# Ouranosinc/xclim

Measured on AMD Instinct MI355X. Metric: grid-cells x timesteps / s (tx90p = percentile_doy + threshold_count + missing mask), higher is better.
Workload: dtype f32

## Files before the change

xclim_amd/csrc/common.h:

```cpp
#pragma once
#include <hip/hip_runtime.h>
#include <stdint.h>
#include <stdio.h>
#include <string.h>

#include "../../include/xclim_hip.h"

struct xh_ctx {
  int device;
  hipStream_t stream;
  hipEvent_t ev0, ev1;
  hipStream_t stream2;
  hipEvent_t ev_ready[2], ev_done[2];
  hipStream_t copy_in, copy_out;
  hipEvent_t ev_lane;
  void* scratch;
  size_t scratch_bytes;
  char* scratch_host;
  size_t scratch_head;
  void* retired[16];
  char* retired_host[16];
  int nretired;
  void* big;
  size_t big_bytes;
// ... 10 lines not shown
  do {                                                                                      \
    hipError_t _e = (expr);                                                                 \
    if (_e != hipSuccess) {                                                                 \
      xh_set_error("%s failed: %s (%s:%d)", #expr, hipGetErrorString(_e), __FILE__, __LINE__); \
      (void)hipGetLastError();   \
      return XH_ERR_HIP;                                                                    \
    }                                                                                       \
  } while (0)

#define XH_REQUIRE(cond, code, ...) \
  do {                              \
    if (!(cond)) {                  \
      xh_set_error(__VA_ARGS__);    \
      return (code);                \
    }                               \
  } while (0)

#define XH_LAUNCH_CHECK()                                                                      \
  do {                                                                                         \
    hipError_t _e = hipGetLastError();                                                         \
    if (_e != hipSuccess) {                                                                    \
      xh_set_error("kernel launch failed: %s (%s:%d)", hipGetErrorString(_e), __FILE__, __LINE__); \
      return XH_ERR_HIP;                                                                       \
    }                                                                                          \
  } while (0)

int xh_nanmax_fix(xh_ctx* ctx, const float* x, int64_t T, int64_t C, int64_t st, int64_t sc, int nq, float* out);
int xh_correction_fix(xh_ctx* ctx, const float* ref, const float* hist, int64_t T, int64_t C, int64_t st, int64_t sc, int nq, int kind,
                      float* af, float* hist_q);
int xh_scratch_upload(xh_ctx* ctx, size_t* cursor, const void* host, size_t bytes, void** dptr);
int xh_big_scratch(xh_ctx* ctx, size_t bytes, void** dptr);
int xh_const_rows(xh_ctx* ctx, int64_t elems, const float** nan_row, const float** ninf_row, const float** pinf_row);
int xh_launch_tcount_doy(xh_ctx* ctx, const float* x, int64_t T, int64_t C, int64_t st, int op, const double* table,
                         int64_t tstride, const int32_t* tidx, const int64_t* d_seg, const int64_t* h_seg, int P, int ndoy,
                         int32_t* count_out, int32_t* valid_out);
int xh_qdm_columns(xh_ctx* ctx, const float* xcols, int64_t T, int64_t ncols, int64_t col_stride, const float* af, int64_t af_qs,
                   const double* d_q, int nq, int kind, int interp, int extrap, float* out, int64_t out_cs);
int xh_qdm_sorted_ws(int64_t T, int64_t ncols, size_t* bytes);
int xh_qdm_sorted(xh_ctx* ctx, const float* xcols, int64_t T, int64_t ncols, int64_t col_stride, const float* af, int64_t af_qs,
                  const double* d_q, int nq, int kind, int interp, int extrap, float* out, int64_t out_cs, void* ws);
int xh_qdm_regsort(xh_ctx* ctx, const float* sim, int64_t T, int64_t C, int64_t st, const float* af, int64_t af_qs,
                   const double* d_q, int nq, int kind, int extrap, float* scen, int64_t ost);
int xh_cut_classify(xh_ctx* ctx, const float* sim, int64_t T, int64_t C, int64_t st, const float* gcut, const float* gfac, int ntest,
                    int kind, float* scen, int64_t ost);
int xh_qdm_hist(xh_ctx* ctx, const float* sim, int64_t T, int64_t C, int64_t st, const float* af, int64_t af_qs, const double* d_q,
                int nq, int kind, int extrap, float* scen, int64_t ost);
int xh_tcount_plan(int64_t T, int64_t C, int64_t st, int op, int P, int ndoy, int64_t longest, size_t* lds, int* narrow);
int64_t xh_tcount_meta_slots(int64_t T);
int64_t xh_tcount_slot_of_row(int64_t t);
int xh_tcount_run(xh_ctx* ctx, const float* x, int64_t T, int64_t C, int64_t st, int op, const double* table, int64_t tstride,
                  const uint32_t* meta, int P, int ndoy, int narrow, size_t lds, int32_t* count_out, int32_t* valid_out);
int xh_select_columns(xh_ctx* ctx, const float* xcols, int64_t T, int64_t ncols, int64_t col_stride, const double* d_q,
                      int nq, float* out, int64_t out_cstride, int64_t out_qstride);
int xh_select_columns_lean(xh_ctx* ctx, const float* xcols, int64_t T, int64_t ncols, int64_t col_stride,
                           const double* d_q, int nq, float* out, int64_t out_cstride, int64_t out_qstride);
int xh_select_columns_radix(xh_ctx* ctx, const float* xcols, int64_t T, int64_t ncols, int64_t col_stride, const double* d_q,
                            int nq, float* out, int64_t out_cstride, int64_t out_qstride);
int xh_select_regsort(xh_ctx* ctx, const float* x, int64_t T, int64_t C, int64_t st, const double* d_q, int nq, float* out,
                      int64_t out_cstride, int64_t out_qstride);
int xh_select_hist(xh_ctx* ctx, const float* x, int64_t T, int64_t C, int64_t st, const double* d_q, int nq, float* out,
                   int64_t out_cstride, int64_t out_qstride);
int xh_select_time_major(xh_ctx* ctx, const float* x, int64_t T, int64_t C, int64_t st, const double* d_q, int nq,
                         float* out, int64_t out_cstride, int64_t out_qstride);

__host__ __device__ static inline int64_t cdiv64(int64_t a, int64_t b) { return (a + b - 1) / b; }

#define XH_BLOCK 256

// ... 212 lines not shown
```

xclim_amd/csrc/quantile.hip:

```cpp
#include <stdlib.h>

#include <type_traits>

#include "pdoy.h"

template <typename Getter>
__device__ __forceinline__ double xh_hf_quantile(int L, int n, double q, double alpha, double beta, Getter get) {
  if (L == 1) return (double)get(0);
  if (n < 2) {
    return n == 1 ? (double)get(0) : xh_nan64();
  }
  double nn = (double)n;
  double vi = nn * q + (alpha + q * (1.0 - alpha - beta)) - 1.0;
  if (vi >= nn - 1.0) return (double)get(n - 1);
  if (vi < 0.0) {
    const float v0 = get(0);
    return (v0 - v0 != 0.0f) ? (double)get(n - 1) : (double)v0;
  }
  double prev = floor(vi);
  int ip = (int)prev;
  double gamma = vi - prev;
  float left = get(ip), right = get(ip + 1);
  float diff = right - left;
  double r = (double)left + (double)diff * gamma;
// ... 67 lines not shown
        return xh_key2f(r);
      };
      for (int j = 0; j < nper; ++j) {
        double r = xh_hf_quantile(N, nvalid[v], qs[j], alpha, beta, get);
        out[((int64_t)j * ndoy + d) * C + c + v] = r;
      }
    }
  }
}

__device__ __forceinline__ void ce(uint32_t& a, uint32_t& b) {
  uint32_t lo = a < b ? a : b, hi = a < b ? b : a;
  a = lo;
  b = hi;
}

template <int W>
__device__ __forceinline__ void sort_small(uint32_t (&k)[W]) {
  if (W == 1) return;
  if (W == 2) { ce(k[0], k[1 % W]); return; }
  if (W == 3) { ce(k[0], k[1 % W]); ce(k[1 % W], k[2 % W]); ce(k[0], k[1 % W]); return; }
  if (W == 5) {
    ce(k[0], k[1 % W]); ce(k[3 % W], k[4 % W]); ce(k[2 % W], k[4 % W]); ce(k[2 % W], k[3 % W]); ce(k[0], k[3 % W]);
    ce(k[0], k[2 % W]); ce(k[1 % W], k[4 % W]); ce(k[1 % W], k[3 % W]); ce(k[1 % W], k[2 % W]);
    return;
  }
#pragma unroll
  for (int r = 0; r < W; ++r) {
#pragma unroll
    for (int i = (r & 1); i + 1 < W; i += 2) ce(k[i], k[i + 1]);
  }
}

template <int W, int VEC, bool COUNT = false>
__global__ void __launch_bounds__(XH_BLOCK)
k_pdoy_slide(const float* __restrict__ x, int64_t T, int64_t C, int64_t st, int64_t t_first, int ndoy, int chunk,
             const QTab* __restrict__ qtab, int nper, double* __restrict__ out, int fast, int op = 0,
             const int32_t* __restrict__ doy_period = nullptr, int32_t* __restrict__ cnt_out = nullptr,
             int32_t* __restrict__ valid_out = nullptr) {
  __shared__ QTab s_tab[8 * (W + 1)];
  for (int i = threadIdx.x; i < nper * (W + 1); i += XH_BLOCK) s_tab[i] = qtab[i];
  __syncthreads();
  constexpr int NP = VEC == 4 ? 2 : 1;
  constexpr int GW = VEC == 4 ? 2 : 1;
  const int lane = threadIdx.x & 63;
  const int64_t wbase = ((int64_t)blockIdx.x * XH_BLOCK + (threadIdx.x & ~63)) * VEC;
  if (wbase >= C) return;
  int64_t cg[NP];
  bool okg[NP];
#pragma unroll
  for (int g = 0; g < NP; ++g) {
    cg[g] = wbase + (VEC == 4 ? 2 * lane + 128 * g : lane);
    okg[g] = cg[g] < C;
  }
  auto cell = [&](int v) -> int64_t { return cg[v / GW] + v % GW; };
  constexpr int half = W / 2;
  int d0 = blockIdx.y * chunk, d1 = d0 + chunk;
  if (d1 > ndoy) d1 = ndoy;
  uint32_t win[VEC][W];
  int n[VEC];
#pragma unroll
  for (int v = 0; v < VEC; ++v) {
    n[v] = 0;
#pragma unroll
    for (int k = 0; k < W; ++k) win[v][k] = 0xFFFFFFFFu;
  }
  auto fetch = [&](int64_t t) -> VecF<VEC> {
    const int64_t tc = t < 0 ? 0 : (t >= T ? T - 1 : t);
    const float* row = x + tc * st;
    VecF<VEC> r;
#pragma unroll
    for (int g = 0; g < NP; ++g) {
      const VecF<GW> h = xh_load<GW>(row + (okg[g] ? cg[g] : C - GW));
#pragma unroll
// ... 499 lines not shown
    hipLaunchKernelGGL((k_pdoy_reg<16, 1>), grid, dim3(XH_BLOCK), 0, ctx->stream, x, T, C, st, d_tbase, nyears, ndoy,
                       window, d_q, nper, alpha, beta, out);
  } else if (N <= 32) {
    dim3 grid((unsigned)cdiv64(C, XH_BLOCK), gy);
    hipLaunchKernelGGL((k_pdoy_reg<32, 1>), grid, dim3(XH_BLOCK), 0, ctx->stream, x, T, C, st, d_tbase, nyears, ndoy,
                       window, d_q, nper, alpha, beta, out);
  } else {
    return launch_pdoy_lds(ctx, x, T, C, st, d_tbase, nyears, ndoy, window, d_q, nper, alpha, beta, out, nullptr, T, nullptr,
                           0);
  }
  XH_LAUNCH_CHECK();
  return XH_OK;
}

static int slide_fast_mode(const QTab* tab, int nper, int W) {
  bool allmax = W > 1, allmin = W > 1;
  for (int j = 0; j < nper; ++j) {
    const QTab& e = tab[j * (W + 1) + W];
    allmax = allmax && e.lo == e.hi && e.lo == W - 1;
    allmin = allmin && e.lo == e.hi && e.lo == 0;
  }
  return allmax ? 1 : (allmin ? 2 : 0);
}

static int pdoy_impl(xh_ctx* ctx, const float* x, int64_t T, int64_t C, int64_t st, const int32_t* tbase, int nyears,
                     int ndoy, int window, const double* qh, int nper, double alpha, double beta, const int32_t* vmap,
                     int64_t Tv, double* out) {
  size_t cur = 0;
  void *d_tb = nullptr, *d_q = nullptr, *d_vmap = nullptr;
  const int N = nyears * window;
  bool contiguous = !vmap && nyears == 1 && nper <= 8 && (window == 3 || window == 5 || window == 7) && tbase[0] >= 0;
  for (int d = 1; contiguous && d < ndoy; ++d) contiguous = tbase[d] == tbase[0] + d;
  if (contiguous) {
    QTab tab[8 * 8];
    build_qtab(window, qh, nper, alpha, beta, tab);
    void* d_tab = nullptr;
    int rc = xh_scratch_upload(ctx, &cur, tab, sizeof(QTab) * (size_t)nper * (window + 1), &d_tab);
    if (rc) return rc;
    int chunk = 32;
    if (const char* e = xh_diag_env("XH_PDOY_SLIDE_CHUNK")) chunk = atoi(e) > 0 ? atoi(e) : chunk;
    const int vec = slide_vec(x, C, st, out);
    dim3 grid((unsigned)cdiv64(cdiv64(C, vec), XH_BLOCK), (unsigned)((ndoy + chunk - 1) / chunk));
#define XH_SLIDE(W, V)                                                                                              \
  hipLaunchKernelGGL((k_pdoy_slide<W, V>), grid, dim3(XH_BLOCK), 0, ctx->stream, x, T, C, st, (int64_t)tbase[0], ndoy, \
                     chunk, (const QTab*)d_tab, nper, out, slide_fast_mode(tab, nper, window))
    if (vec == 4) {
      if (window == 3) XH_SLIDE(3, 4); else if (window == 5) XH_SLIDE(5, 4); else XH_SLIDE(7, 4);
    } else {
      if (window == 3) XH_SLIDE(3, 1); else if (window == 5) XH_SLIDE(5, 1); else XH_SLIDE(7, 1);
    }
#undef XH_SLIDE
    XH_LAUNCH_CHECK();
    return XH_OK;
  }
  int rc = xh_scratch_upload(ctx, &cur, tbase, sizeof(int32_t) * (size_t)nyears * ndoy, &d_tb);
  if (rc) return rc;
  rc = xh_scratch_upload(ctx, &cur, qh, sizeof(double) * nper, &d_q);
  if (rc) return rc;
  if (vmap) {
    rc = xh_scratch_upload(ctx, &cur, vmap, sizeof(int32_t) * (size_t)Tv, &d_vmap);
    if (rc) return rc;
  }
  if (!vmap && N <= 32)
    return launch_pdoy(ctx, x, T, C, st, (const int32_t*)d_tb, nyears, ndoy, window, (const double*)d_q, nper, alpha, beta,
                       out);
  const bool mergeable = N > 32 && nyears <= 64 && (window == 3 || window == 5 || window == 7) && nper <= 16;
  if (!mergeable)
    return launch_pdoy_lds(ctx, x, T, C, st, (const int32_t*)d_tb, nyears, ndoy, window, (const double*)d_q, nper, alpha,
                           beta, out, (const int32_t*)d_vmap, Tv, nullptr, 0);
  uint8_t* regular = (uint8_t*)malloc((size_t)ndoy);
  int32_t* irregular = (int32_t*)malloc(sizeof(int32_t) * (size_t)ndoy);
  QTab* tab = (QTab*)malloc(sizeof(QTab) * (size_t)nper * (N + 1));
  if (!regular || !irregular || !tab) {
    free(regular); free(irregular); free(tab);
    xh_set_error("xh_percentile_doy: out of host memory");
    return XH_ERR_ARG;
  }
  const int nirr = pdoy_regular_flags(tbase, nyears, ndoy, window, T, vmap, Tv, regular, irregular);
// ... 76 lines not shown
                                         hipFuncAttributeMaxDynamicSharedMemorySize, (int)lds));                           \
      hipLaunchKernelGGL((k_pdoy_merge<W, NY, false>), grid, dim3(64), lds, ctx->stream, x, T, C, st, (const int32_t*)d_tb, \
                         nyears, ndoy, chunk, (const QTab*)d_tab, (const int32_t*)d_jrest, nrest, out,                      \
                         (const int32_t*)d_vmap, Tv, (const uint8_t*)d_reg, (const int32_t*)nullptr, 0, KT, KB, abl);       \
    }                                                                                                                      \
    if (nirr) {                                                                                                            \
      if (lds_a > 64 * 1024)                                                                                               \
        XH_CHECK_HIP(hipFuncSetAttribute((const void*)k_pdoy_merge<W, NY, true>,                                           \
                                         hipFuncAttributeMaxDynamicSharedMemorySize, (int)lds_a));                         \
      hipLaunchKernelGGL((k_pdoy_merge<W, NY, true>), grid_irr, dim3(64), lds_a, ctx->stream, x, T, C, st,                  \
                         (const int32_t*)d_tb, nyears, ndoy, chunk, (const QTab*)d_tab, (const int32_t*)d_jall, nper, out,  \
                         (const int32_t*)d_vmap, Tv, (const uint8_t*)d_reg, (const int32_t*)d_irr, nirr, KTa, KBa, abl);    \
    }                                                                                                                      \
  } while (0)
  if (NYP == 32) {
    if (window == 3) XH_MERGE(3, 32); else if (window == 5) XH_MERGE(5, 32); else XH_MERGE(7, 32);
  } else {
    if (window == 3) XH_MERGE(3, 64); else if (window == 5) XH_MERGE(5, 64); else XH_MERGE(7, 64);
  }
#undef XH_MERGE
  XH_LAUNCH_CHECK();
  return XH_OK;
}

static int pdoy_count_impl(xh_ctx* ctx, const float* x, int64_t T, int64_t C, int64_t st, const int32_t* tbase, int ndoy,
                           int window, double per, double alpha, double beta, int op, const int32_t* doy_period, int P,
                           int32_t* count_out, int32_t* valid_out) {
  bool contiguous = (window == 3 || window == 5 || window == 7) && tbase[0] >= 0;
  for (int d = 1; contiguous && d < ndoy; ++d) contiguous = tbase[d] == tbase[0] + d;
  if (!contiguous) return XH_ERR_NOTIMPL;
  for (int d = 0; d < ndoy; ++d)
    XH_REQUIRE(doy_period[d] >= 0 && doy_period[d] < P, XH_ERR_ARG, "xh_percentile_doy_count: doy_period[%d] outside [0, P)", d);
  size_t cur = 0;
  QTab tab[8];
  const double q = per / 100.0;
  build_qtab(window, &q, 1, alpha, beta, tab);
  void *d_tab = nullptr, *d_dp = nullptr;
  int rc = xh_scratch_upload(ctx, &cur, tab, sizeof(QTab) * (size_t)(window + 1), &d_tab);
  if (!rc) rc = xh_scratch_upload(ctx, &cur, doy_period, sizeof(int32_t) * (size_t)ndoy, &d_dp);
  if (rc) return rc;
  XH_CHECK_HIP(hipMemsetAsync(count_out, 0, sizeof(int32_t) * (size_t)P * (size_t)C, ctx->stream));
  if (valid_out) XH_CHECK_HIP(hipMemsetAsync(valid_out, 0, sizeof(int32_t) * (size_t)P * (size_t)C, ctx->stream));
  int chunk = 61;
  if (const char* e = xh_diag_env("XH_PDOY_SLIDE_COUNT_CHUNK")) chunk = atoi(e) > 0 ? atoi(e) : chunk;
  const int vec = slide_vec(x, C, st, nullptr);
  dim3 grid((unsigned)cdiv64(cdiv64(C, vec), XH_BLOCK), (unsigned)((ndoy + chunk - 1) / chunk));
#define XH_SLIDEC(W, V)                                                                                                   \
  hipLaunchKernelGGL((k_pdoy_slide<W, V, true>), grid, dim3(XH_BLOCK), 0, ctx->stream, x, T, C, st, (int64_t)tbase[0], ndoy, \
                     chunk, (const QTab*)d_tab, 1, (double*)nullptr, slide_fast_mode(tab, 1, window), op,          \
                     (const int32_t*)d_dp, count_out, valid_out)
  if (vec == 4) {
    if (window == 3) XH_SLIDEC(3, 4); else if (window == 5) XH_SLIDEC(5, 4); else XH_SLIDEC(7, 4);
  } else {
    if (window == 3) XH_SLIDEC(3, 1); else if (window == 5) XH_SLIDEC(5, 1); else XH_SLIDEC(7, 1);
  }
#undef XH_SLIDEC
  XH_LAUNCH_CHECK();
  return XH_OK;
}

static int pdoy_count_multi(xh_ctx* ctx, const float* x, int64_t T, int64_t C, int64_t st, const int32_t* tbase, int nyears,
                            int ndoy, int window, double per, double alpha, double beta, int op, const int32_t* doy_period,
                            int P, int32_t* count_out, int32_t* valid_out) {
  const int N = nyears * window;
  if (!(N > 32 && nyears <= 64 && (window == 3 || window == 5 || window == 7))) return XH_ERR_NOTIMPL;
  if (op != XH_OP_GT && op != XH_OP_GE && op != XH_OP_LT && op != XH_OP_LE) return XH_ERR_NOTIMPL;
  for (int64_t i = 0; i < (int64_t)nyears * ndoy; ++i) {
    XH_REQUIRE(tbase[i] >= -1 && tbase[i] < T, XH_ERR_ARG, "xh_percentile_doy_count: tbase entry out of range");
    XH_REQUIRE(tbase[i] < 0 ? doy_period[i] < 0 : (doy_period[i] >= 0 && doy_period[i] < P), XH_ERR_ARG,
               "xh_percentile_doy_count: doy_period[%lld] must be in [0, P) for present days and < 0 for absent ones",
               (long long)i);
  }
  uint8_t* regular = (uint8_t*)malloc((size_t)ndoy);
  int32_t* irregular = (int32_t*)malloc(sizeof(int32_t) * (size_t)ndoy);
  QTab* tab = (QTab*)malloc(sizeof(QTab) * (size_t)(N + 1));
  if (!regular || !irregular || !tab) {
    free(regular); free(irregular); free(tab);
    xh_set_error("xh_percentile_doy_count: out of host memory");
    return XH_ERR_ARG;
  }
  const int nirr = pdoy_regular_flags(tbase, nyears, ndoy, window, T, nullptr, T, regular, irregular);
  const double q = per / 100.0;
// ... 188 lines not shown
```

xclim_amd/csrc/reduce.hip:

```cpp
#include "common.h"
#include "window.h"

template <int VEC, int KIND>
__global__ void __launch_bounds__(XH_BLOCK)
k_threshold_count(const float* __restrict__ x, int64_t C, int64_t st, int op, float thr32, double thr64,
                  const void* __restrict__ table, int64_t tstride, const int32_t* __restrict__ tidx,
                  const int64_t* __restrict__ seg_off, int P, int32_t* __restrict__ count_out,
                  int32_t* __restrict__ valid_out, int period_fast) {
  const unsigned tile = period_fast ? blockIdx.y : blockIdx.x;
  const int pstart = period_fast ? blockIdx.x : blockIdx.y, pstep = period_fast ? gridDim.x : gridDim.y;
  int64_t c = ((int64_t)tile * XH_BLOCK + threadIdx.x) * VEC;
  if (c >= C) return;
  for (int p = pstart; p < P; p += pstep) {
    int64_t t0 = seg_off[p], t1 = seg_off[p + 1];
    int cnt[VEC], val[VEC];
#pragma unroll
    for (int i = 0; i < VEC; ++i) cnt[i] = 0, val[i] = 0;
    xh_march_rows<VEC, 8>(x + c, st, t0, t1, [&](int64_t t, const VecF<VEC>& xv) {
      if (KIND == XH_THR_SCALAR_F32) {
#pragma unroll
        for (int i = 0; i < VEC; ++i) cnt[i] += xh_cmp_f32(xv.v[i], op, thr32) ? 1 : 0;
      } else if (KIND == XH_THR_SCALAR_F64) {
#pragma unroll
        for (int i = 0; i < VEC; ++i) cnt[i] += xh_cmp_f64((double)xv.v[i], op, thr64) ? 1 : 0;
// ... 170 lines not shown
        else if (RED == XH_RED_VAR) r = (poisoned || n[i] == 0) ? xh_nan32() : (float)(s2[i] / (double)n[i]);
        else r = (poisoned || n[i] == 0) ? xh_nan32() : (float)sqrt(s2[i] / (double)n[i]);
        if (len == 0 && RED != XH_RED_SUM) r = xh_nan32();
        reinterpret_cast<float*>(out_v)[o + i] = r;
      }
    }
    if (valid_out) {
#pragma unroll
      for (int i = 0; i < VEC; ++i) valid_out[o + i] = n[i];
    }
  }
}

template <int VEC>
static int launch_resample_reduce(xh_ctx* ctx, int reducer, dim3 grid, const float* x, int64_t C, int64_t st, int skipna,
                                  const int64_t* seg, int P, void* out, int32_t* valid_out) {
#define XH_RR(R)                                                                                                   \
  case R:                                                                                                          \
    hipLaunchKernelGGL((k_resample_reduce<VEC, R>), grid, dim3(XH_BLOCK), 0, ctx->stream, x, C, st, skipna, seg, P, out, \
                       valid_out);                                                                                 \
    break;
  switch (reducer) {
    XH_RR(XH_RED_SUM) XH_RR(XH_RED_MEAN) XH_RR(XH_RED_MIN) XH_RR(XH_RED_MAX) XH_RR(XH_RED_STD) XH_RR(XH_RED_VAR)
    XH_RR(XH_RED_COUNT) XH_RR(XH_RED_ARGMIN) XH_RR(XH_RED_ARGMAX)
    default:
      xh_set_error("xh_resample_reduce: reducer %d not recognized", reducer);
      return XH_ERR_OP;
  }
#undef XH_RR
  XH_LAUNCH_CHECK();
  return XH_OK;
}

__global__ void __launch_bounds__(XH_BLOCK)
k_apply_missing_mask(const void* __restrict__ value, int kind, const int32_t* __restrict__ valid,
                     const int32_t* __restrict__ expected, int P, int64_t C, double* __restrict__ out) {
  int64_t i = (int64_t)blockIdx.x * XH_BLOCK + threadIdx.x;
  int64_t n = (int64_t)P * C;
  if (i >= n) return;
  int p = (int)(i / C);
  double v = kind == 0 ? (double)reinterpret_cast<const int32_t*>(value)[i]
             : kind == 1 ? (double)reinterpret_cast<const float*>(value)[i]
                         : reinterpret_cast<const double*>(value)[i];
  out[i] = (valid[i] != expected[p]) ? xh_nan64() : v;
}

template <int RED>
__global__ void __launch_bounds__(XH_BLOCK)
k_rolling_reduce(const float* __restrict__ x, int64_t T, int64_t C, int64_t st, int window, int left, int right,
                 float* __restrict__ out, int64_t out_st) {
  int64_t c = (int64_t)blockIdx.x * XH_BLOCK + threadIdx.x;
  if (c >= C) return;
  int64_t chunk = cdiv64(T, (int64_t)gridDim.y);
  int64_t ta = (int64_t)blockIdx.y * chunk, tb = ta + chunk;
  if (tb > T) tb = T;
  for (int64_t t = ta; t < tb; ++t) {
    int64_t a = t - left, b = t + right;
    float r;
    if (RED == XH_RED_COUNT) {
      int n = 0;
      for (int64_t k = (a < 0 ? 0 : a); k <= b && k < T; ++k) {
        float v = x[k * st + c];
        n += (v == v) ? 1 : 0;
      }
      r = (float)n;
    } else if (a < 0 || b >= T) {
      r = xh_nan32();
    } else {
      double s = 0.0;
      float e = x[a * st + c];
      bool nan = false;
      for (int64_t k = a; k <= b; ++k) {
        float v = x[k * st + c];
        nan |= (v != v);
        if (RED == XH_RED_MIN) e = v < e ? v : e;
        else if (RED == XH_RED_MAX) e = v > e ? v : e;
        else s += (double)v;
      }
      if (RED == XH_RED_SUM) r = (float)s;
      else if (RED == XH_RED_MEAN) r = (float)(s / (double)window);
      else if (RED == XH_RED_MIN || RED == XH_RED_MAX) r = e;
      else {
        double m = s / (double)window, s2 = 0.0;
        for (int64_t k = a; k <= b; ++k) {
          double d = (double)x[k * st + c] - m;
          s2 += d * d;
        }
        r = (RED == XH_RED_VAR) ? (float)(s2 / (double)window) : (float)sqrt(s2 / (double)window);
      }
      if (nan) r = xh_nan32();
    }
    out[t * out_st + c] = r;
  }
}

static int check_tc(const char* fn, xh_ctx* ctx, const void* x, int64_t T, int64_t C, int64_t st, int64_t sc) {
  XH_REQUIRE(ctx && x, XH_ERR_ARG, "%s: NULL argument", fn);
  XH_REQUIRE(T >= 0 && C >= 0, XH_ERR_ARG, "%s: negative shape", fn);
  XH_REQUIRE(sc == 1 && st >= C, XH_ERR_LAYOUT,
             "%s: streaming kernels need a time-major view (sc == 1, st >= C); got st=%lld sc=%lld — transpose first",
             fn, (long long)st, (long long)sc);
  return XH_OK;
}

static int upload_segments(xh_ctx* ctx, size_t* cur, const int64_t* seg_off, int P, int64_t T, const char* fn,
                           const int64_t** d_seg) {
  XH_REQUIRE(seg_off && P >= 1, XH_ERR_ARG, "%s: seg_off NULL or P < 1", fn);
  for (int p = 0; p < P; ++p)
    XH_REQUIRE(seg_off[p] <= seg_off[p + 1] && seg_off[p] >= 0 && seg_off[p + 1] <= T, XH_ERR_ARG,
               "%s: seg_off must be non-decreasing within [0, T]", fn);
  void* d = nullptr;
  int rc = xh_scratch_upload(ctx, cur, seg_off, sizeof(int64_t) * (size_t)(P + 1), &d);
  if (rc) return rc;
  *d_seg = (const int64_t*)d;
  return XH_OK;
}

extern "C" {

static int threshold_count_impl(xh_ctx* ctx, const float* x, int64_t T, int64_t C, int64_t st, int64_t sc, int op, int thr_kind,
                                double thr_scalar, const void* thr_table, int64_t thr_stride, const int32_t* tidx,
                                const int64_t* seg_off, int P, int32_t* count_out, int32_t* valid_out, int ndoy) {
  int rc = check_tc("xh_threshold_count", ctx, x, T, C, st, sc);
  if (rc) return rc;
  XH_REQUIRE(op >= XH_OP_GT && op <= XH_OP_NE, XH_ERR_OP, "Operation `%d` not recognized.", op);
  XH_REQUIRE(count_out, XH_ERR_ARG, "xh_threshold_count: count_out is NULL");
  if (thr_kind >= XH_THR_DOY_F64) {
    XH_REQUIRE(thr_table && thr_stride >= C, XH_ERR_ARG, "xh_threshold_count: threshold table missing or stride < C");
    if (thr_kind == XH_THR_DOY_F64 || thr_kind == XH_THR_DOY_F32)
      XH_REQUIRE(tidx, XH_ERR_ARG, "xh_threshold_count: tidx required for per-doy thresholds");
  }
  size_t cur = 0;
  const int64_t* d_seg = nullptr;
  rc = upload_segments(ctx, &cur, seg_off, P, T, "xh_threshold_count", &d_seg);
  if (rc) return rc;
  if (C == 0) return XH_OK;
  if (thr_kind == XH_THR_DOY_F64 && ndoy > 0 && !xh_diag_env("XH_TCOUNT_LEGACY")) {
    rc = xh_launch_tcount_doy(ctx, x, T, C, st, op, static_cast<const double*>(thr_table), thr_stride, tidx, d_seg, seg_off, P,
                              ndoy, count_out, valid_out);
    if (rc != XH_ERR_NOTIMPL) return rc;
  }
  int vec = xh_pick_vec(x, C, st);
  if (thr_kind >= XH_THR_DOY_F64) {
    size_t esz = (thr_kind == XH_THR_DOY_F64 || thr_kind == XH_THR_FULL_F64) ? 8 : 4;
    if ((reinterpret_cast<uintptr_t>(thr_table) & 15) != 0 || (thr_stride * esz) % 16 != 0) vec = 1;
  }
  unsigned tiles = (unsigned)cdiv64(cdiv64(C, vec), XH_BLOCK);
  const bool doy = thr_kind == XH_THR_DOY_F64 || thr_kind == XH_THR_DOY_F32;
  const int period_fast = (doy && P > 1 && tiles <= 65535u) ? 1 : 0;
  dim3 grid = period_fast ? dim3(period_grid(P), tiles) : dim3(tiles, period_grid(P));
  if (vec == 4)
    return launch_threshold_count<4>(ctx, thr_kind, grid, x, C, st, op, thr_scalar, thr_table, thr_stride, tidx, d_seg, P,
                                     count_out, valid_out, period_fast);
  return launch_threshold_count<1>(ctx, thr_kind, grid, x, C, st, op, thr_scalar, thr_table, thr_stride, tidx, d_seg, P,
                                   count_out, valid_out, period_fast);
}

int xh_threshold_count(xh_ctx* ctx, const float* x, int64_t T, int64_t C, int64_t st, int64_t sc, int op, int thr_kind,
                       double thr_scalar, const void* thr_table, int64_t thr_stride, const int32_t* tidx,
                       const int64_t* seg_off, int P, int32_t* count_out, int32_t* valid_out) {
  return threshold_count_impl(ctx, x, T, C, st, sc, op, thr_kind, thr_scalar, thr_table, thr_stride, tidx, seg_off, P, count_out,
                              valid_out, 0);
}

int xh_threshold_count_doy(xh_ctx* ctx, const float* x, int64_t T, int64_t C, int64_t st, int64_t sc, int op,
                           const double* thr_table, int64_t thr_stride, int ndoy, const int32_t* tidx, const int64_t* seg_off,
                           int P, int32_t* count_out, int32_t* valid_out) {
  XH_REQUIRE(ndoy >= 1, XH_ERR_ARG, "xh_threshold_count_doy: the table needs at least one row (ndoy = %d)", ndoy);
  return threshold_count_impl(ctx, x, T, C, st, sc, op, XH_THR_DOY_F64, 0.0, thr_table, thr_stride, tidx, seg_off, P, count_out,
                              valid_out, ndoy);
}

int xh_domain_count(xh_ctx* ctx, const float* x, int64_t T, int64_t C, int64_t st, int64_t sc, int op1, double thr1,
                    int op2, double thr2, int combine, const int64_t* seg_off, int P, int32_t* count_out,
// ... 19 lines not shown
    hipLaunchKernelGGL((k_domain_count<4, true>), grid, dim3(XH_BLOCK), 0, ctx->stream, x, C, st, s1, c1.thr, s2, c2.thr, combine,
                       d_seg, P, count_out, valid_out);
  } else if (vec == 4)
    hipLaunchKernelGGL((k_domain_count<4>), grid, dim3(XH_BLOCK), 0, ctx->stream, x, C, st, op1, (float)thr1, op2,
                       (float)thr2, combine, d_seg, P, count_out, valid_out);
  else
    hipLaunchKernelGGL((k_domain_count<1>), grid, dim3(XH_BLOCK), 0, ctx->stream, x, C, st, op1, (float)thr1, op2,
                       (float)thr2, combine, d_seg, P, count_out, valid_out);
  XH_LAUNCH_CHECK();
  return XH_OK;
}

int xh_resample_reduce(xh_ctx* ctx, const float* x, int64_t T, int64_t C, int64_t st, int64_t sc, int reducer, int skipna,
                       const int64_t* seg_off, int P, void* out, int32_t* valid_out) {
  int rc = check_tc("xh_resample_reduce", ctx, x, T, C, st, sc);
  if (rc) return rc;
  XH_REQUIRE(out, XH_ERR_ARG, "xh_resample_reduce: out is NULL");
  size_t cur = 0;
  const int64_t* d_seg = nullptr;
  rc = upload_segments(ctx, &cur, seg_off, P, T, "xh_resample_reduce", &d_seg);
  if (rc) return rc;
  if (C == 0) return XH_OK;
  int vec = xh_pick_vec(x, C, st);
  dim3 grid((unsigned)cdiv64(cdiv64(C, vec), XH_BLOCK), period_grid(P));
  if (vec == 4) return launch_resample_reduce<4>(ctx, reducer, grid, x, C, st, skipna, d_seg, P, out, valid_out);
  return launch_resample_reduce<1>(ctx, reducer, grid, x, C, st, skipna, d_seg, P, out, valid_out);
}

int xh_apply_missing_mask(xh_ctx* ctx, const void* value, int value_kind, const int32_t* valid, const int32_t* expected,
                          int P, int64_t C, double* out64) {
  XH_REQUIRE(ctx && value && valid && expected && out64, XH_ERR_ARG, "xh_apply_missing_mask: NULL argument");
  XH_REQUIRE(value_kind >= 0 && value_kind <= 2, XH_ERR_ARG, "xh_apply_missing_mask: value_kind must be 0, 1 or 2");
  XH_REQUIRE(P >= 1 && C >= 0, XH_ERR_ARG, "xh_apply_missing_mask: bad shape");
  size_t cur = 0;
  void* d_exp = nullptr;
  int rc = xh_scratch_upload(ctx, &cur, expected, sizeof(int32_t) * (size_t)P, &d_exp);
  if (rc) return rc;
  int64_t n = (int64_t)P * C;
  if (n == 0) return XH_OK;
  hipLaunchKernelGGL(k_apply_missing_mask, dim3((unsigned)cdiv64(n, XH_BLOCK)), dim3(XH_BLOCK), 0, ctx->stream, value,
                     value_kind, valid, (const int32_t*)d_exp, P, C, out64);
  XH_LAUNCH_CHECK();
  return XH_OK;
}

int xh_rolling_reduce(xh_ctx* ctx, const float* x, int64_t T, int64_t C, int64_t st, int64_t sc, int window, int center,
                      int reducer, float* out, int64_t out_st) {
  int rc = check_tc("xh_rolling_reduce", ctx, x, T, C, st, sc);
  if (rc) return rc;
  XH_REQUIRE(out && out_st >= C, XH_ERR_ARG, "xh_rolling_reduce: out NULL or out_st < C");
  XH_REQUIRE(window >= 1, XH_ERR_ARG, "xh_rolling_reduce: window must be >= 1");
  if (T == 0 || C == 0) return XH_OK;
  int left = center ? window / 2 : window - 1;
  int right = window - 1 - left;
  {
    int rr = xh_launch_rolling_ring(ctx, x, T, C, st, window, left, right, reducer, out, out_st);
    if (rr != XH_ERR_NOTIMPL) return rr;
  }
  unsigned ny = (unsigned)(T < 64 ? T : 64);
  dim3 grid((unsigned)cdiv64(C, XH_BLOCK), ny);
#define XH_RO(R)                                                                                                      \
  case R:                                                                                                             \
    hipLaunchKernelGGL((k_rolling_reduce<R>), grid, dim3(XH_BLOCK), 0, ctx->stream, x, T, C, st, window, left, right, out, \
                       out_st);                                                                                       \
    break;
  switch (reducer) {
    XH_RO(XH_RED_SUM) XH_RO(XH_RED_MEAN) XH_RO(XH_RED_MIN) XH_RO(XH_RED_MAX) XH_RO(XH_RED_STD) XH_RO(XH_RED_VAR)
    XH_RO(XH_RED_COUNT)
    default:
      xh_set_error("xh_rolling_reduce: reducer %d not recognized", reducer);
      return XH_ERR_OP;
  }
#undef XH_RO
  XH_LAUNCH_CHECK();
// ... 5 lines not shown
```

xclim_amd/csrc/tcount.hip:

```cpp
#include "f32thr.h"
#include "rowstream.h"

namespace {

constexpr int TC_CW = 64, TC_RL = 16, TC_U = 16, TC_NT = TC_CW * TC_RL, TC_ROWS = TC_RL * TC_U;

__global__ void k_tc_meta(const int32_t* __restrict__ tidx, const int64_t* __restrict__ seg, int P, int64_t T, int64_t nslots,
                          int ndoy, uint32_t* __restrict__ meta) {
  const int64_t i = (int64_t)blockIdx.x * blockDim.x + threadIdx.x;
  if (i >= nslots) return;
  const int64_t kb = i >> 8;
  const int rl = (int)(i >> 4) & 15, u = (int)i & 15;
  const int64_t t = kb * TC_ROWS + u * TC_RL + rl;
  uint32_t dy = (uint32_t)ndoy, per = (uint32_t)P;
  if (t < T) {
    const int d = tidx[t];
    if (d >= 0 && d < ndoy) dy = (uint32_t)d;
    if (t >= seg[0] && t < seg[P]) {
      int lo = 0, hi = P;
      while (hi - lo > 1) {
        const int mid = (lo + hi) >> 1;
        if (seg[mid] <= t) lo = mid; else hi = mid;
      }
      per = (uint32_t)lo;
// ... 115 lines not shown

int64_t xh_tcount_slot_of_row(int64_t t) {
  const int64_t kb = t / TC_ROWS, r = t % TC_ROWS;
  return (kb * TC_RL + r % TC_RL) * TC_U + r / TC_RL;
}

int xh_tcount_run(xh_ctx* ctx, const float* x, int64_t T, int64_t C, int64_t st, int op, const double* table, int64_t tstride,
                  const uint32_t* meta, int P, int ndoy, int narrow, size_t lds, int32_t* count_out, int32_t* valid_out) {
  const int64_t ntiles = cdiv64(C, TC_CW);
  const unsigned grid = (unsigned)(ntiles < ctx->num_cu ? ntiles : ctx->num_cu);
#define XH_TCD2(OPV, NW)                                                                                                      \
  {                                                                                                                           \
    XH_CHECK_HIP(hipFuncSetAttribute((const void*)k_tc_doy<OPV, NW>, hipFuncAttributeMaxDynamicSharedMemorySize, (int)lds)); \
    hipLaunchKernelGGL((k_tc_doy<OPV, NW>), dim3(grid), dim3(TC_NT), lds, ctx->stream, x, (int)T, C, st, table, tstride, meta,  \
                       ndoy, P, count_out, valid_out);                                                                        \
  }
#define XH_TCD(OPV)                         \
  case OPV:                                 \
    if (narrow) XH_TCD2(OPV, true) else XH_TCD2(OPV, false) \
    break;
  switch (op) {
    XH_TCD(XH_OP_GT)
    XH_TCD(XH_OP_LT)
    XH_TCD(XH_OP_GE)
    XH_TCD(XH_OP_LE)
  }
#undef XH_TCD2
#undef XH_TCD
  XH_LAUNCH_CHECK();
  return XH_OK;
}

int xh_launch_tcount_doy(xh_ctx* ctx, const float* x, int64_t T, int64_t C, int64_t st, int op, const double* table,
                         int64_t tstride, const int32_t* tidx, const int64_t* d_seg, const int64_t* h_seg, int P, int ndoy,
                         int32_t* count_out, int32_t* valid_out) {
  int64_t longest = 0;
  for (int p = 0; p < P; ++p) longest = h_seg[p + 1] - h_seg[p] > longest ? h_seg[p + 1] - h_seg[p] : longest;
  size_t lds = 0;
  int narrow = 0;
  int rc = xh_tcount_plan(T, C, st, op, P, ndoy, longest, &lds, &narrow);
  if (rc) return rc;
  const int64_t nslots = xh_tcount_meta_slots(T);
  void* scratch = nullptr;
  rc = xh_big_scratch(ctx, (size_t)nslots * 4, &scratch);
  if (rc) return rc;
  uint32_t* meta = static_cast<uint32_t*>(scratch);
  hipLaunchKernelGGL(k_tc_meta, dim3((unsigned)cdiv64(nslots, 256)), dim3(256), 0, ctx->stream, tidx, d_seg, P, T, nslots, ndoy, meta);
  return xh_tcount_run(ctx, x, T, C, st, op, table, tstride, meta, P, ndoy, narrow, lds, count_out, valid_out);
}
```

Before: 229.7 billion.

## Pass small tables as kernel arguments and add streaming per-year threshold count kernel

Small quantile tables and the expected-count array for the missing mask are now passed by value as kernel arguments instead of being uploaded to scratch memory. Segment offsets are uploaded only inside the doy tcount path. A new fallback kernel counts threshold exceedances by streaming rows in double-buffered batches with segment bounds held in kernel arguments. The aim is to remove host-to-device uploads and sync overhead on small inputs and to give a faster fallback when the LDS-based doy kernel declines. In exchange, kernel argument size grows and more specialised kernel variants are built.

```diff
diff --git a/xclim_amd/csrc/common.h b/xclim_amd/csrc/common.h
--- a/xclim_amd/csrc/common.h
+++ b/xclim_amd/csrc/common.h
@@ -66,8 +66,8 @@
 int xh_big_scratch(xh_ctx* ctx, size_t bytes, void** dptr);
 int xh_const_rows(xh_ctx* ctx, int64_t elems, const float** nan_row, const float** ninf_row, const float** pinf_row);
 int xh_launch_tcount_doy(xh_ctx* ctx, const float* x, int64_t T, int64_t C, int64_t st, int op, const double* table,
-                         int64_t tstride, const int32_t* tidx, const int64_t* d_seg, const int64_t* h_seg, int P, int ndoy,
-                         int32_t* count_out, int32_t* valid_out);
+                         int64_t tstride, const int32_t* tidx, const int64_t* h_seg, int P, int ndoy, int32_t* count_out,
+                         int32_t* valid_out);
 int xh_qdm_columns(xh_ctx* ctx, const float* xcols, int64_t T, int64_t ncols, int64_t col_stride, const float* af, int64_t af_qs,
                    const double* d_q, int nq, int kind, int interp, int extrap, float* out, int64_t out_cs);
 int xh_qdm_sorted_ws(int64_t T, int64_t ncols, size_t* bytes);
diff --git a/xclim_amd/csrc/quantile.hip b/xclim_amd/csrc/quantile.hip
--- a/xclim_amd/csrc/quantile.hip
+++ b/xclim_amd/csrc/quantile.hip
@@ -123,14 +123,18 @@
   }
 }
 
+struct SlideTab {
+  QTab e[8 * 8];
+};
+
 template <int W, int VEC, bool COUNT = false>
 __global__ void __launch_bounds__(XH_BLOCK)
 k_pdoy_slide(const float* __restrict__ x, int64_t T, int64_t C, int64_t st, int64_t t_first, int ndoy, int chunk,
-             const QTab* __restrict__ qtab, int nper, double* __restrict__ out, int fast, int op = 0,
+             const SlideTab qtab, int nper, double* __restrict__ out, int fast, int op = 0,
              const int32_t* __restrict__ doy_period = nullptr, int32_t* __restrict__ cnt_out = nullptr,
              int32_t* __restrict__ valid_out = nullptr) {
   __shared__ QTab s_tab[8 * (W + 1)];
-  for (int i = threadIdx.x; i < nper * (W + 1); i += XH_BLOCK) s_tab[i] = qtab[i];
+  for (int i = threadIdx.x; i < nper * (W + 1); i += XH_BLOCK) s_tab[i] = qtab.e[i];
   __syncthreads();
   constexpr int NP = VEC == 4 ? 2 : 1;
   constexpr int GW = VEC == 4 ? 2 : 1;
@@ -696,18 +700,17 @@
   bool contiguous = !vmap && nyears == 1 && nper <= 8 && (window == 3 || window == 5 || window == 7) && tbase[0] >= 0;
   for (int d = 1; contiguous && d < ndoy; ++d) contiguous = tbase[d] == tbase[0] + d;
   if (contiguous) {
-    QTab tab[8 * 8];
+    SlideTab st8;
+    memset(&st8, 0, sizeof(st8));
+    QTab* tab = st8.e;
     build_qtab(window, qh, nper, alpha, beta, tab);
-    void* d_tab = nullptr;
-    int rc = xh_scratch_upload(ctx, &cur, tab, sizeof(QTab) * (size_t)nper * (window + 1), &d_tab);
-    if (rc) return rc;
     int chunk = 32;
     if (const char* e = xh_diag_env("XH_PDOY_SLIDE_CHUNK")) chunk = atoi(e) > 0 ? atoi(e) : chunk;
     const int vec = slide_vec(x, C, st, out);
     dim3 grid((unsigned)cdiv64(cdiv64(C, vec), XH_BLOCK), (unsigned)((ndoy + chunk - 1) / chunk));
 #define XH_SLIDE(W, V)                                                                                              \
   hipLaunchKernelGGL((k_pdoy_slide<W, V>), grid, dim3(XH_BLOCK), 0, ctx->stream, x, T, C, st, (int64_t)tbase[0], ndoy, \
-                     chunk, (const QTab*)d_tab, nper, out, slide_fast_mode(tab, nper, window))
+                     chunk, st8, nper, out, slide_fast_mode(tab, nper, window))
     if (vec == 4) {
       if (window == 3) XH_SLIDE(3, 4); else if (window == 5) XH_SLIDE(5, 4); else XH_SLIDE(7, 4);
     } else {
@@ -850,12 +853,13 @@
   for (int d = 0; d < ndoy; ++d)
     XH_REQUIRE(doy_period[d] >= 0 && doy_period[d] < P, XH_ERR_ARG, "xh_percentile_doy_count: doy_period[%d] outside [0, P)", d);
   size_t cur = 0;
-  QTab tab[8];
+  SlideTab st8;
+  memset(&st8, 0, sizeof(st8));
+  QTab* tab = st8.e;
   const double q = per / 100.0;
   build_qtab(window, &q, 1, alpha, beta, tab);
-  void *d_tab = nullptr, *d_dp = nullptr;
-  int rc = xh_scratch_upload(ctx, &cur, tab, sizeof(QTab) * (size_t)(window + 1), &d_tab);
-  if (!rc) rc = xh_scratch_upload(ctx, &cur, doy_period, sizeof(int32_t) * (size_t)ndoy, &d_dp);
+  void* d_dp = nullptr;
+  int rc = xh_scratch_upload(ctx, &cur, doy_period, sizeof(int32_t) * (size_t)ndoy, &d_dp);
   if (rc) return rc;
   XH_CHECK_HIP(hipMemsetAsync(count_out, 0, sizeof(int32_t) * (size_t)P * (size_t)C, ctx->stream));
   if (valid_out) XH_CHECK_HIP(hipMemsetAsync(valid_out, 0, sizeof(int32_t) * (size_t)P * (size_t)C, ctx->stream));
@@ -865,7 +869,7 @@
   dim3 grid((unsigned)cdiv64(cdiv64(C, vec), XH_BLOCK), (unsigned)((ndoy + chunk - 1) / chunk));
 #define XH_SLIDEC(W, V)                                                                                                   \
   hipLaunchKernelGGL((k_pdoy_slide<W, V, true>), grid, dim3(XH_BLOCK), 0, ctx->stream, x, T, C, st, (int64_t)tbase[0], ndoy, \
-                     chunk, (const QTab*)d_tab, 1, (double*)nullptr, slide_fast_mode(tab, 1, window), op,          \
+                     chunk, st8, 1, (double*)nullptr, slide_fast_mode(tab, 1, window), op,          \
                      (const int32_t*)d_dp, count_out, valid_out)
   if (vec == 4) {
     if (window == 3) XH_SLIDEC(3, 4); else if (window == 5) XH_SLIDEC(5, 4); else XH_SLIDEC(7, 4);
diff --git a/xclim_amd/csrc/reduce.hip b/xclim_amd/csrc/reduce.hip
--- a/xclim_amd/csrc/reduce.hip
+++ b/xclim_amd/csrc/reduce.hip
@@ -226,9 +226,14 @@
   return XH_OK;
 }
 
+#define XH_MASK_SMALL 64
+struct XhMaskExp {
+  int32_t v[XH_MASK_SMALL];
+};
 __global__ void __launch_bounds__(XH_BLOCK)
 k_apply_missing_mask(const void* __restrict__ value, int kind, const int32_t* __restrict__ valid,
-                     const int32_t* __restrict__ expected, int P, int64_t C, double* __restrict__ out) {
+                     const int32_t* __restrict__ expected, const XhMaskExp exp_small, int P, int64_t C,
+                     double* __restrict__ out) {
   int64_t i = (int64_t)blockIdx.x * XH_BLOCK + threadIdx.x;
   int64_t n = (int64_t)P * C;
   if (i >= n) return;
@@ -236,7 +241,8 @@
   double v = kind == 0 ? (double)reinterpret_cast<const int32_t*>(value)[i]
              : kind == 1 ? (double)reinterpret_cast<const float*>(value)[i]
                          : reinterpret_cast<const double*>(value)[i];
-  out[i] = (valid[i] != expected[p]) ? xh_nan64() : v;
+  const int32_t e = expected ? expected[p] : exp_small.v[p];
+  out[i] = (valid[i] != e) ? xh_nan64() : v;
 }
 
 template <int RED>
@@ -297,18 +303,28 @@
   return XH_OK;
 }
 
-static int upload_segments(xh_ctx* ctx, size_t* cur, const int64_t* seg_off, int P, int64_t T, const char* fn,
-                           const int64_t** d_seg) {
+static int check_segments(const int64_t* seg_off, int P, int64_t T, const char* fn) {
   XH_REQUIRE(seg_off && P >= 1, XH_ERR_ARG, "%s: seg_off NULL or P < 1", fn);
   for (int p = 0; p < P; ++p)
     XH_REQUIRE(seg_off[p] <= seg_off[p + 1] && seg_off[p] >= 0 && seg_off[p + 1] <= T, XH_ERR_ARG,
                "%s: seg_off must be non-decreasing within [0, T]", fn);
+  return XH_OK;
+}
+
+static int upload_segments(xh_ctx* ctx, size_t* cur, const int64_t* seg_off, int P, int64_t T, const char* fn,
+                           const int64_t** d_seg) {
+  int rc = check_segments(seg_off, P, T, fn);
+  if (rc) return rc;
   void* d = nullptr;
-  int rc = xh_scratch_upload(ctx, cur, seg_off, sizeof(int64_t) * (size_t)(P + 1), &d);
+  rc = xh_scratch_upload(ctx, cur, seg_off, sizeof(int64_t) * (size_t)(P + 1), &d);
   if (rc) return rc;
   *d_seg = (const int64_t*)d;
   return XH_OK;
 }
+
+__attribute__((weak)) int xh_launch_tcount_year(xh_ctx* ctx, const float* x, int64_t T, int64_t C, int64_t st, int op,
+                                                const double* table, int64_t tstride, const int32_t* tidx,
+                                                const int64_t* seg_off, int P, int32_t* count_out, int32_t* valid_out);
 
 extern "C" {
 
@@ -324,16 +340,24 @@
     if (thr_kind == XH_THR_DOY_F64 || thr_kind == XH_THR_DOY_F32)
       XH_REQUIRE(tidx, XH_ERR_ARG, "xh_threshold_count: tidx required for per-doy thresholds");
   }
+  rc = check_segments(seg_off, P, T, "xh_threshold_count");
+  if (rc) return rc;
+  if (C == 0) return XH_OK;
+  const bool legacy = xh_diag_env("XH_TCOUNT_LEGACY") != nullptr;
+  if (thr_kind == XH_THR_DOY_F64 && ndoy > 0 && !legacy) {
+    rc = xh_launch_tcount_doy(ctx, x, T, C, st, op, static_cast<const double*>(thr_table), thr_stride, tidx, seg_off, P, ndoy,
+                              count_out, valid_out);
+    if (rc != XH_ERR_NOTIMPL) return rc;
+  }
+  if (thr_kind == XH_THR_DOY_F64 && !legacy && xh_launch_tcount_year) {
+    rc = xh_launch_tcount_year(ctx, x, T, C, st, op, static_cast<const double*>(thr_table), thr_stride, tidx, seg_off, P,
+                               count_out, valid_out);
+    if (rc != XH_ERR_NOTIMPL) return rc;
+  }
   size_t cur = 0;
   const int64_t* d_seg = nullptr;
   rc = upload_segments(ctx, &cur, seg_off, P, T, "xh_threshold_count", &d_seg);
   if (rc) return rc;
-  if (C == 0) return XH_OK;
-  if (thr_kind == XH_THR_DOY_F64 && ndoy > 0 && !xh_diag_env("XH_TCOUNT_LEGACY")) {
-    rc = xh_launch_tcount_doy(ctx, x, T, C, st, op, static_cast<const double*>(thr_table), thr_stride, tidx, d_seg, seg_off, P,
-                              ndoy, count_out, valid_out);
-    if (rc != XH_ERR_NOTIMPL) return rc;
-  }
   int vec = xh_pick_vec(x, C, st);
   if (thr_kind >= XH_THR_DOY_F64) {
     size_t esz = (thr_kind == XH_THR_DOY_F64 || thr_kind == XH_THR_FULL_F64) ? 8 : 4;
@@ -419,14 +443,20 @@
   XH_REQUIRE(ctx && value && valid && expected && out64, XH_ERR_ARG, "xh_apply_missing_mask: NULL argument");
   XH_REQUIRE(value_kind >= 0 && value_kind <= 2, XH_ERR_ARG, "xh_apply_missing_mask: value_kind must be 0, 1 or 2");
   XH_REQUIRE(P >= 1 && C >= 0, XH_ERR_ARG, "xh_apply_missing_mask: bad shape");
-  size_t cur = 0;
+  XhMaskExp small;
+  memset(&small, 0, sizeof(small));
   void* d_exp = nullptr;
-  int rc = xh_scratch_upload(ctx, &cur, expected, sizeof(int32_t) * (size_t)P, &d_exp);
-  if (rc) return rc;
+  if (P <= XH_MASK_SMALL) {
+    memcpy(small.v, expected, sizeof(int32_t) * (size_t)P);
+  } else {
+    size_t cur = 0;
+    int rc = xh_scratch_upload(ctx, &cur, expected, sizeof(int32_t) * (size_t)P, &d_exp);
+    if (rc) return rc;
+  }
   int64_t n = (int64_t)P * C;
   if (n == 0) return XH_OK;
   hipLaunchKernelGGL(k_apply_missing_mask, dim3((unsigned)cdiv64(n, XH_BLOCK)), dim3(XH_BLOCK), 0, ctx->stream, value,
-                     value_kind, valid, (const int32_t*)d_exp, P, C, out64);
+                     value_kind, valid, (const int32_t*)d_exp, small, P, C, out64);
   XH_LAUNCH_CHECK();
   return XH_OK;
 }
diff --git a/xclim_amd/csrc/tcount.hip b/xclim_amd/csrc/tcount.hip
--- a/xclim_amd/csrc/tcount.hip
+++ b/xclim_amd/csrc/tcount.hip
@@ -171,19 +171,23 @@
 }
 
 int xh_launch_tcount_doy(xh_ctx* ctx, const float* x, int64_t T, int64_t C, int64_t st, int op, const double* table,
-                         int64_t tstride, const int32_t* tidx, const int64_t* d_seg, const int64_t* h_seg, int P, int ndoy,
-                         int32_t* count_out, int32_t* valid_out) {
+                         int64_t tstride, const int32_t* tidx, const int64_t* h_seg, int P, int ndoy, int32_t* count_out,
+                         int32_t* valid_out) {
   int64_t longest = 0;
   for (int p = 0; p < P; ++p) longest = h_seg[p + 1] - h_seg[p] > longest ? h_seg[p + 1] - h_seg[p] : longest;
   size_t lds = 0;
   int narrow = 0;
   int rc = xh_tcount_plan(T, C, st, op, P, ndoy, longest, &lds, &narrow);
   if (rc) return rc;
+  size_t cur = 0;
+  void* d_seg = nullptr;
+  rc = xh_scratch_upload(ctx, &cur, h_seg, sizeof(int64_t) * (size_t)(P + 1), &d_seg);
+  if (rc) return rc;
   const int64_t nslots = xh_tcount_meta_slots(T);
   void* scratch = nullptr;
   rc = xh_big_scratch(ctx, (size_t)nslots * 4, &scratch);
   if (rc) return rc;
   uint32_t* meta = static_cast<uint32_t*>(scratch);
-  hipLaunchKernelGGL(k_tc_meta, dim3((unsigned)cdiv64(nslots, 256)), dim3(256), 0, ctx->stream, tidx, d_seg, P, T, nslots, ndoy, meta);
+  hipLaunchKernelGGL(k_tc_meta, dim3((unsigned)cdiv64(nslots, 256)), dim3(256), 0, ctx->stream, tidx, (const int64_t*)d_seg, P, T, nslots, ndoy, meta);
   return xh_tcount_run(ctx, x, T, C, st, op, table, tstride, meta, P, ndoy, narrow, lds, count_out, valid_out);
 }
diff --git a/xclim_amd/csrc/tcyear.hip b/xclim_amd/csrc/tcyear.hip
--- /dev/null
+++ b/xclim_amd/csrc/tcyear.hip
@@ -0,0 +1,162 @@
+#include "common.h"
+
+namespace {
+
+constexpr int TY_MAXP = 64;
+
+struct TySeg {
+  int32_t v[TY_MAXP + 1];
+};
+
+template <int OP, int NP, int R, bool REV>
+__global__ void __launch_bounds__(XH_BLOCK)
+k_tc_year(const float* __restrict__ x, int64_t C, int64_t st, const double* __restrict__ table, int64_t tstride,
+          const int32_t* __restrict__ tidx, const TySeg seg, int P, int32_t* __restrict__ count_out,
+          int32_t* __restrict__ valid_out) {
+  constexpr int V = 2 * NP;
+  const int lane = threadIdx.x & 63;
+  const int64_t wbase = ((int64_t)blockIdx.x * XH_BLOCK + __builtin_amdgcn_readfirstlane(threadIdx.x & ~63)) * V;
+  if (wbase >= C) return;
+  int64_t cg[NP];
+  uint32_t offx[NP], offt[NP];
+  bool okg[NP];
+#pragma unroll
+  for (int g = 0; g < NP; ++g) {
+    cg[g] = wbase + 2 * lane + 128 * g;
+    okg[g] = cg[g] < C;
+    const int64_t cc = okg[g] ? cg[g] : C - 2;
+    offx[g] = (uint32_t)(cc * 4);
+    offt[g] = (uint32_t)(cc * 8);
+  }
+  const int tB = seg.v[0], tE = seg.v[P];
+  constexpr int DIR = REV ? -1 : 1;
+  int p = REV ? P - 1 : 0;
+  int tlim = REV ? seg.v[__builtin_amdgcn_readfirstlane(P - 1)] : seg.v[1];
+  auto outside = [&](int t) { return REV ? t < tlim : t >= tlim; };
+  int cnt[V], val[V];
+#pragma unroll
+  for (int v = 0; v < V; ++v) cnt[v] = 0, val[v] = 0;
+  auto flush = [&]() {
+#pragma unroll
+    for (int g = 0; g < NP; ++g) {
+      if (!okg[g]) continue;
+      const int64_t o = (int64_t)p * C + cg[g];
+      *reinterpret_cast<int2*>(count_out + o) = make_int2(cnt[2 * g], cnt[2 * g + 1]);
+      if (valid_out) *reinterpret_cast<int2*>(valid_out + o) = make_int2(val[2 * g], val[2 * g + 1]);
+    }
+#pragma unroll
+    for (int v = 0; v < V; ++v) cnt[v] = 0, val[v] = 0;
+    p += DIR;
+    if (REV) tlim = p >= 0 ? seg.v[__builtin_amdgcn_readfirstlane(p)] : tB;
+    else tlim = p < P ? seg.v[__builtin_amdgcn_readfirstlane(p + 1)] : tE;
+  };
+  auto more_periods = [&]() { return REV ? p >= 0 : p < P; };
+  if (tE <= tB) {
+    while (more_periods()) flush();
+    return;
+  }
+
+  struct Batch {
+    float2 xs[R][NP];
+    double2 th[R][NP];
+  };
+  auto rowc = [&](int t) { return REV ? (t >= tB ? t : tB) : (t < tE ? t : tE - 1); };
+  auto fetch_doys = [&](int tb, int (&d)[R]) {
+#pragma unroll
+    for (int u = 0; u < R; ++u) d[u] = tidx[rowc(tb + DIR * u)];
+  };
+  auto issue = [&](int tb, const int (&d)[R], Batch& b) {
+#pragma unroll
+    for (int u = 0; u < R; ++u) {
+      const char* xr = reinterpret_cast<const char*>(x + (int64_t)rowc(tb + DIR * u) * st);
+      const char* tr = reinterpret_cast<const char*>(table + (int64_t)d[u] * tstride);
+#pragma unroll
+      for (int g = 0; g < NP; ++g) {
+        b.xs[u][g] = *reinterpret_cast<const float2*>(xr + offx[g]);
+        b.th[u][g] = *reinterpret_cast<const double2*>(tr + offt[g]);
+      }
+    }
+  };
+  auto consume = [&](int tb, const Batch& b) {
+#pragma unroll
+    for (int u = 0; u < R; ++u) {
+      const int t = tb + DIR * u;
+      if (REV ? t < tB : t >= tE) break;
+      while (outside(t)) flush();
+#pragma unroll
+      for (int g = 0; g < NP; ++g) {
+        const float a0 = b.xs[u][g].x, a1 = b.xs[u][g].y;
+        cnt[2 * g] += xh_cmp_f64((double)a0, OP, b.th[u][g].x) ? 1 : 0;
+        cnt[2 * g + 1] += xh_cmp_f64((double)a1, OP, b.th[u][g].y) ? 1 : 0;
+        val[2 * g] += (a0 == a0) ? 1 : 0;
+        val[2 * g + 1] += (a1 == a1) ? 1 : 0;
+      }
+    }
+  };
+
+  Batch A, B;
+  int dA[R], dB[R];
+  const int t0 = REV ? tE - 1 : tB;
+  fetch_doys(t0, dA);
+  issue(t0, dA, A);
+  fetch_doys(t0 + DIR * R, dB);
+  const int nb = (tE - tB + R - 1) / R;
+  for (int b = 0; b < nb; b += 2) {
+    const int ta = t0 + DIR * b * R;
+    issue(ta + DIR * R, dB, B);
+    fetch_doys(ta + DIR * 2 * R, dA);
+    consume(ta, A);
+    issue(ta + DIR * 2 * R, dA, A);
+    fetch_doys(ta + DIR * 3 * R, dB);
+    consume(ta + DIR * R, B);
+  }
+  while (more_periods()) flush();
+}
+
+template <int NP, int R, bool REV>
+static void launch_geom(xh_ctx* ctx, int op, dim3 grid, const float* x, int64_t C, int64_t st, const double* table,
+                        int64_t tstride, const int32_t* tidx, const TySeg& seg, int P, int32_t* count_out,
+                        int32_t* valid_out) {
+#define XH_TY(OP)                                                                                                       \
+  case OP:                                                                                                              \
+    hipLaunchKernelGGL((k_tc_year<OP, NP, R, REV>), grid, dim3(XH_BLOCK), 0, ctx->stream, x, C, st, table, tstride, tidx, seg, \
+                       P, count_out, valid_out);                                                                        \
+    break;
+  switch (op) {
+    XH_TY(XH_OP_GT) XH_TY(XH_OP_LT) XH_TY(XH_OP_GE) XH_TY(XH_OP_LE) XH_TY(XH_OP_EQ) XH_TY(XH_OP_NE)
+  }
+#undef XH_TY
+}
+
+}
+
+int xh_launch_tcount_year(xh_ctx* ctx, const float* x, int64_t T, int64_t C, int64_t st, int op, const double* table,
+                          int64_t tstride, const int32_t* tidx, const int64_t* seg_off, int P, int32_t* count_out,
+                          int32_t* valid_out) {
+  if (op < XH_OP_GT || op > XH_OP_NE || P < 1 || P > TY_MAXP || T >= ((int64_t)1 << 31)) return XH_ERR_NOTIMPL;
+  if (xh_pick_vec(x, C, st) != 4) return XH_ERR_NOTIMPL;
+  if ((reinterpret_cast<uintptr_t>(table) & 15) != 0 || (tstride * 8) % 16 != 0) return XH_ERR_NOTIMPL;
+  if (C * 4 >= ((int64_t)1 << 32) || C * 8 >= ((int64_t)1 << 32)) return XH_ERR_NOTIMPL;
+  TySeg seg;
+  for (int p = 0; p <= P; ++p) seg.v[p] = (int32_t)seg_off[p];
+  for (int p = P + 1; p <= TY_MAXP; ++p) seg.v[p] = seg.v[P];
+  if (C == 0) return XH_OK;
+  int np = 2, r = 4, rev = 1;
+  if (const char* e = xh_diag_env("XH_TCYEAR_GEOM")) {
+    int a = 0, b = 0, c = 1;
+    if (sscanf(e, "%d,%d,%d", &a, &b, &c) >= 2 && (a == 1 || a == 2) && (b == 4 || b == 8)) np = a, r = b, rev = c != 0;
+  }
+  const dim3 grid((unsigned)cdiv64(C, (int64_t)XH_BLOCK * 2 * np));
+#define XH_TYG(NPV, RV, REVV) \
+  launch_geom<NPV, RV, REVV>(ctx, op, grid, x, C, st, table, tstride, tidx, seg, P, count_out, valid_out)
+  if (rev) {
+    if (np == 2 && r == 4) XH_TYG(2, 4, true); else if (np == 2) XH_TYG(2, 8, true);
+    else if (r == 4) XH_TYG(1, 4, true); else XH_TYG(1, 8, true);
+  } else {
+    if (np == 2 && r == 4) XH_TYG(2, 4, false); else if (np == 2) XH_TYG(2, 8, false);
+    else if (r == 4) XH_TYG(1, 4, false); else XH_TYG(1, 8, false);
+  }
+#undef XH_TYG
+  XH_LAUNCH_CHECK();
+  return XH_OK;
+}
```

New measurement: 229.3 billion (median of 6 runs). Within noise of the previous version (-0.2%).
